# karenyang/GCN-VAE

Hardware: AMD Instinct MI355X
Metric: edges/sec R-GCN forward+backward, FB15k-237 emb=200 (higher is better)
Workload: dtype f32; 1 GPU; FB15k-237-shaped synthetic full graph (BASELINE configs[1]): 14541 entities, 474 directed relation types, E=544230 directed edges on this rank (544230 in the trained graph), 2-layer R-GCN-VAE bdd num_bases=100 emb_dim=200 dropout 0.2, 0 IAF blocks, DistMult decoder on T=220000 triplets per rank, step = fwd + loss(BCE+reg+KL+MMD) + bwd + clip + Adam; edges_per_gpu=544230, trained_graph_edges=544230, nodes=14541, triplets_per_gpu=220000, n_flows=0, gemm_precision=f32, launch=hipgraph, parallelism=single GPU, optimizer=replicated clip + Adam, k1_operands=f32

## Files before the change

### gcn-vae_amd/csrc/k_loss.hip

```cpp
#include "common.h"

namespace gv {

constexpr int RED_BLOCKS = 1024;

__device__ __forceinline__ float block_sum_256(float v, float* sm ) {
    v = wave_sum(v);
    const int lane = threadIdx.x & 63, w = threadIdx.x >> 6;
    __syncthreads();
    if (lane == 0) sm[w] = v;
    __syncthreads();
    return sm[0] + sm[1] + sm[2] + sm[3];
}

__global__ __launch_bounds__(256) void k_final_sum(const float* part, int n, float scale, float* out, int accumulate) {
    __shared__ float sm[4];
    float acc = 0.f;
    for (int i = threadIdx.x; i < n; i += 256) acc += part[i];
    const float tot = block_sum_256(acc, sm);
    if (threadIdx.x == 0) *out = accumulate ? *out + scale * tot : scale * tot;
}

__global__ __launch_bounds__(256) void k_loss_combine(const float* p0, int n0, float s0, const float* p1, int n1, float s1,
                                                      const float* p2, int n2, float s2, const float* p3, int n3, float s3,
// ... 1001 lines not shown
        } else {
            *reinterpret_cast<float4*>(o + 4 * q) = s4;
        }
    }
}

__global__ __launch_bounds__(256) void k_prior_sample_fwd(const float* z_pre, const float* eps, float* out, int s, int k, int h) {
    const int total = s * h;
    for (int i = blockIdx.x * 256 + threadIdx.x; i < total; i += gridDim.x * 256) {
        const int r = i / h, c = i - r * h, j = r % k;
        const float v = softplus_t(z_pre[(size_t)(k + j) * h + c]) + 1e-8f;
        out[i] = z_pre[(size_t)j * h + c] + eps[i] * sqrtf(v);
    }
}

__global__ __launch_bounds__(256) void k_prior_sample_bwd(const float* z_pre, const float* eps, const float* g, float* gz_pre,
                                                          int accumulate, int s, int k, int h) {
    const int total = k * h;
    for (int i = blockIdx.x * 256 + threadIdx.x; i < total; i += gridDim.x * 256) {
        const int j = i / h, c = i - j * h;
        const float raw = z_pre[(size_t)(k + j) * h + c];
        const float v = softplus_t(raw) + 1e-8f;
        float gm = 0.f, gs = 0.f;
        for (int r = j; r < s; r += k) {
            gm += g[(size_t)r * h + c];
            gs += g[(size_t)r * h + c] * eps[(size_t)r * h + c];
        }
        const float gr = gs * 0.5f / sqrtf(v) * (raw > 20.f ? 1.f : 1.f / (1.f + expf(-raw)));
        gz_pre[i] = accumulate ? gz_pre[i] + gm : gm;
        gz_pre[total + i] = accumulate ? gz_pre[total + i] + gr : gr;
    }
}

constexpr int KL_SLICES = 256;
constexpr int KL_FUSED_KT = 16;

}

using namespace gv;

#define GV_ST ((hipStream_t)stream)

static int red_blocks(int64_t n, int per_block) {
    int64_t b = (n + per_block - 1) / per_block;
    return (int)(b < 1 ? 1 : (b > RED_BLOCKS ? RED_BLOCKS : b));
}

static int sq2_blocks(int64_t n, int cap) {
    const int b = red_blocks(n, 4096);
    return b > cap ? cap : b;
}

static int kl_blocks(int64_t n) { return (int)((n + 3) / 4 > RED_BLOCKS ? RED_BLOCKS : (n + 3) / 4); }

extern "C" int gv_distmult_bce_fwd(const float* embed, int ld_e, const float* w_rel, int ld_w,
                                   const int32_t* triplets, const int32_t* order, const float* labels, const float* bias,
                                   float* score, float* loss, float* workspace, int64_t t, int h, void* stream) {
    GV_REQUIRE(embed && w_rel && triplets && labels && score && workspace, GV_ERR_NULL,
               "gv_distmult_bce_fwd: NULL pointer");
    GV_REQUIRE(t > 0 && h > 0 && ld_e >= h && ld_w >= h, GV_ERR_SHAPE, "gv_distmult_bce_fwd: bad shape");
    const int nb = red_blocks(t, 16);
    hipLaunchKernelGGL(k_distmult_bce, dim3(nb), dim3(256), 0, GV_ST, embed, ld_e, w_rel, ld_w, triplets, order, labels,
                       bias, score, workspace, t, h);
    if (loss) hipLaunchKernelGGL(k_final_sum, dim3(1), dim3(256), 0, GV_ST, workspace, nb, 1.f / (float)t, loss, 0);
    return launch_status("gv_distmult_bce_fwd");
}
// ... 250 lines not shown
    const float* kl_part = ws_kl ? ws_kl + 3 * (size_t)k * h : nullptr;
    hipLaunchKernelGGL(k_loss_combine, dim3(1), dim3(256), 0, GV_ST, ws_pred, n0, 1.f / (float)t, ws_reg, n1, 1.f, kl_part,
                       n2, ws_kl ? 1.f / (float)n_nodes : 0.f, ws_mmd, n3, 1.f, reg_w, kl_w, mmd_w, scal, loss, rows_dev,
                       (float)n_nodes);
    return launch_status("gv_loss_combine");
}

extern "C" int gv_mmd_bwd(const float* x, const float* y, const int64_t* y_index, int sx, int sy, int h, const float* gmmd,
                          float gscale, float* gx, float* gy, void* stream) {
    GV_REQUIRE(x && y && gx && gy, GV_ERR_NULL, "gv_mmd_bwd: NULL pointer");
    GV_REQUIRE(sx > 0 && sy > 0 && h > 0 && h <= 1024, GV_ERR_SHAPE, "gv_mmd_bwd: bad shape");
    static const int v2 = getenv("GV_MMD_ROWS16") ? atoi(getenv("GV_MMD_ROWS16")) : 1;
    const bool al = h % 4 == 0 && aligned16(x) && aligned16(y) && aligned16(gx) && aligned16(gy);
    if (v2 && al && h <= 256) hipLaunchKernelGGL(k_mmd_bwd_g<4>, dim3(sx + sy), dim3(64 * MMD_WAVES), 0, GV_ST, x, y, y_index, sx, sy, h, gmmd, gscale, gx, gy);
    else if (h <= 256) hipLaunchKernelGGL(k_mmd_bwd<4>, dim3(sx + sy), dim3(64 * MMD_WAVES), 0, GV_ST, x, y, y_index, sx, sy, h, gmmd, gscale, gx, gy);
    else hipLaunchKernelGGL(k_mmd_bwd<16>, dim3(sx + sy), dim3(64 * MMD_WAVES), 0, GV_ST, x, y, y_index, sx, sy, h, gmmd, gscale, gx, gy);
    return launch_status("gv_mmd_bwd");
}

extern "C" int gv_prior_sample_fwd(const float* z_pre, const float* eps, float* out, int s, int k, int h, void* stream) {
    GV_REQUIRE(z_pre && eps && out, GV_ERR_NULL, "gv_prior_sample_fwd: NULL pointer");
    GV_REQUIRE(s > 0 && k > 0 && h > 0, GV_ERR_SHAPE, "gv_prior_sample_fwd: bad shape");
    hipLaunchKernelGGL(k_prior_sample_fwd, dim3((s * h + 255) / 256), dim3(256), 0, GV_ST, z_pre, eps, out, s, k, h);
    return launch_status("gv_prior_sample_fwd");
}

extern "C" int gv_prior_sample_bwd(const float* z_pre, const float* eps, const float* g, float* gz_pre, int accumulate,
                                   int s, int k, int h, void* stream) {
    GV_REQUIRE(z_pre && eps && g && gz_pre, GV_ERR_NULL, "gv_prior_sample_bwd: NULL pointer");
    GV_REQUIRE(s > 0 && k > 0 && h > 0, GV_ERR_SHAPE, "gv_prior_sample_bwd: bad shape");
    hipLaunchKernelGGL(k_prior_sample_bwd, dim3((k * h + 255) / 256), dim3(256), 0, GV_ST, z_pre, eps, g, gz_pre, accumulate, s, k, h);
    return launch_status("gv_prior_sample_bwd");
}
```

### gcn-vae_amd/lib.py

```python
import ctypes
import os

import torch

_HERE = os.path.dirname(os.path.abspath(__file__))
LIB_PATH = os.path.join(_HERE, 'libgcnvae_hip.so')

_P, _I, _L, _F = ctypes.c_void_p, ctypes.c_int, ctypes.c_int64, ctypes.c_float

SIGNATURES = {
    'gv_version': (_I, []),
    'gv_last_error_string': (ctypes.c_char_p, []),
    'gv_index_caps': (None, [_L, _I, _I, _P, _P, _P]),
    'gv_index_workspace_bytes': (_L, [_L, _I]),
    'gv_build_csr': (_I, [_P, _L, _I, _I, _P, _P, _P, _I, _P, _I, _P, _L, _P]),
    'gv_build_csr_batch_workspace_bytes': (_L, [_P, _I]),
    'gv_build_csr_batch': (_I, [_P, _I, _P, _L, _P]),
    'gv_triplet_lists': (_I, [_P, _I, _L, _P, _P, _P, _P, _P, _P, _P, _P, _P]),
    'gv_widen2_i32': (_I, [_P, _P, _L, _P, _P, _L, _P]),
    'gv_graph_index_build': (_I, [_P, _P, _L, _I, _I, _I, _I, _P, _P, _P, _P, _I, _P, _I, _P, _P, _P, _P, _I, _P, _I, _P, _L, _P]),
    'gv_relation_index_build': (_I, [_P, _P, _P, _P, _P, _L, _I, _I, _P, _P, _P, _P, _P, _P, _P, _I, _P, _I, _P, _L, _P]),
    'gv_triplet_index_build': (_I, [_P, _L, _I, _I, _I, _I, _P, _P, _P, _P, _P, _I, _P, _I, _P, _P, _P, _P, _P, _I, _P, _I,
                                    _P, _L, _P]),
    'gv_perm_sample': (_I, [_L, _L, ctypes.c_uint64, ctypes.c_uint64, _P, _P, ctypes.c_uint32, _P, _P]),
# ... 76 lines not shown
    'gv_rank_scores': (_I, [_P, _I, _P, _I, _P, _P, _P, _P, _I, _I, _I, _P]),
    'gv_rank_scores_filtered': (_I, [_P, _I, _P, _I, _P, _P, _P, _P, _P, _I, _P, _P, _P, _I, _I, _I, _P]),
    'gv_topk_scores_workspace_bytes': (_L, [_I, _I, _I]),
    'gv_topk_scores': (_I, [_P, _I, _P, _I, _P, _P, _P, _P, _I, _I, _P, _P, _P, _I, _I, _I, _P]),
    'gv_rank_scores_constrained': (_I, [_P, _I, _P, _I, _P, _P, _P, _P, _P, _I, _P, _I, _I, _P, _P, _P, _P, _P, _P, _I, _I, _I, _P]),
    'gv_topk_scores_constrained': (_I, [_P, _I, _P, _I, _P, _P, _P, _P, _I, _P, _I, _I, _P, _I, _P, _P, _P, _I, _I, _I, _P]),
    'gv_mine_scores_workspace_bytes': (_L, [_I, _I, _I]),
    'gv_mine_scores': (_I, [_P, _I, _P, _I, _P, _P, _P, _P, _I, _I, _I, ctypes.c_uint32, _I, ctypes.c_uint32, _I, _P, _L, _P, _P, _P, _L,
                            _I, _I, _I, _P]),
    'gv_ec_basis_rows_fwd': (_I, [_P, _P, _P, _P, _L, _I, _I, _I, _L, _P, _P]),
    'gv_ec_basis_rows_bwd': (_I, [_P, _P, _P, _P, _P, _P, _L, _P, _P, _L, _I, _I, _I, _L, _P, _P, _P, _I, _P]),
    'gv_ec_head_fwd': (_I, [_P, _P, _P, _P, _L, _I, _P, _P, _P, _P, _P, _P]),
    'gv_ec_head_bwd': (_I, [_P, _P, _P, _P, _P, _P, _L, _I, _P, _P]),
    'gv_transe_sample': (_I, [_P, ctypes.c_uint32, _P, _L, _I, _P, _P, _P, _P, _P, _I, _I, _P, _P, _P, _P, _P]),
    'gv_transe_step': (_I, [_P, _P, _P, _P, _P, _I, _I, _I, _I, _I, _F, _F, _F, _P, _P, _P, _P, _P, _P]),
    'gv_transe_apply': (_I, [_P, _I, _P, _P, _P, _P, _I, _P, _P, _P, _I, _F, _P, _I, _F, _P, _P, _P]),
    'gv_transe_queries': (_I, [_P, _P, _P, _P, _L, _I, _I, _I, _P, _P]),
    'gv_transe_distances': (_I, [_P, _L, _P, _I, _I, _I, _P, _P]),
    'gv_transe_rank_filtered': (_I, [_P, _L, _P, _I, _I, _I, _P, _P, _P, _P, _P, _P, _P]),
    'gv_transe_topk_workspace_bytes': (_L, [_L, _I, _I]),
    'gv_transe_topk': (_I, [_P, _L, _P, _I, _I, _I, _P, _P, _P, _I, _I, _P, _P, _P, _P]),
    'gv_transe_rank_constrained': (_I, [_P, _L, _P, _I, _I, _I, _P, _P, _P, _P, _P, _I, _I, _P, _P, _P, _P, _P, _P]),
    'gv_transe_topk_constrained': (_I, [_P, _L, _P, _I, _I, _I, _P, _P, _P, _I, _P, _I, _I, _P, _I, _P, _P, _P, _P]),
    'gv_colsum': (_I, [_P, _P, _L, _I, _I, _P, _P, _I, _P]),
    'gv_gather_rows': (_I, [_P, _P, _P, _L, _I, _P]),
    'gv_gather_rows_rng_tick': (_I, [_P, _P, _P, _L, _I, _P, _P]),
    'gv_rng_fill': (_I, [_P, _I, _P, _P, _P, _P, _P, _P]),
    'gv_rng_tick': (_I, [_P, _P]),
    'gv_scatter_add_rows': (_I, [_P, _P, _P, _L, _I, _P]),
    'gv_reparam_fwd': (_I, [_P, _P, _P, _P, _P, _L, _I, _P]),
    'gv_reparam_bwd': (_I, [_P, _P, _P, _P, _P, _P, _P, _L, _I, _P]),
    'gv_distmult_bce_fwd': (_I, [_P, _I, _P, _I, _P, _P, _P, _P, _P, _P, _P, _L, _I, _P]),
    'gv_bce_grad': (_I, [_P, _P, _P, _P, _P, _P, _P, _P, _P, _L, _P]),
    'gv_mean_sq': (_I, [_P, _L, _F, _P, _P, _I, _P]),
    'gv_mean_sq2': (_I, [_P, _L, _F, _P, _L, _F, _P, _P, _P, _L, _P]),
    'gv_axpby': (_I, [_L, _P, _F, _P, _F, _P, _P]),
    'gv_mul': (_I, [_L, _P, _P, _P, _P]),
    'gv_mul_multi': (_I, [_I, _P, _P, _P, _P, _P]),
    'gv_kl_workspace_bytes': (_L, [_L, _I, _I]),
    'gv_kl_fwd': (_I, [_P, _P, _I, _P, _P, _P, _P, _P, _P, _L, _I, _I, _P, _P]),
    'gv_kl_bwd': (_I, [_P, _P, _I, _P, _P, _P, _P, _F, _F, _P, _P, _P, _P, _I, _P, _I, _L, _I, _I, _P, _P]),
    'gv_reparam_kl_fwd': (_I, [_P, _P, _P, _P, _P, _P, _P, _P, _L, _I, _I, _P]),
    'gv_reparam_kl_bwd': (_I, [_P, _P, _P, _P, _P, _P, _P, _F, _F, _P, _P, _P, _I, _P, _L, _I, _I, _P]),
    'gv_loss_combine': (_I, [_P, _L, _P, _L, _L, _P, _L, _I, _I, _P, _I, _I, _F, _F, _F, _P, _P, _P, _P]),
    'gv_lincomb4': (_I, [_P, _F, _P, _F, _P, _F, _P, _F, _P, _P]),
    'gv_mmd_fwd': (_I, [_P, _P, _P, _I, _I, _I, _P, _P, _P]),
    'gv_mmd_bwd': (_I, [_P, _P, _P, _I, _I, _I, _P, _F, _P, _P, _P]),
    'gv_prior_sample_fwd': (_I, [_P, _P, _P, _I, _I, _I, _P]),
    'gv_prior_sample_bwd': (_I, [_P, _P, _P, _P, _I, _I, _I, _I, _P]),
    'gv_iaf_update_fwd': (_I, [_P, _P, _I, _P, _P, _P, _L, _I, _P]),
    'gv_iaf_update_bwd': (_I, [_P, _P, _I, _P, _P, _P, _P, _P, _P, _L, _I, _P]),
    'gv_iaf_update_bwd_acc': (_I, [_P, _P, _I, _P, _P, _P, _P, _I, _P, _P, _L, _I, _P]),
    'gv_rowsum': (_I, [_P, _I, _I, _I, _P, _L, _P]),
    'gv_reverse_cols': (_I, [_P, _P, _L, _I, _P]),
    'gv_mean_rows_multi': (_I, [_I, _P, _L, _P, _P, _P, _P]),
    'gv_mean_rows_bwd': (_I, [_P, _L, _L, _P, _P, _P]),
    'gv_adam_step': (_I, [_P, _P, _P, _P, _L, _P, _F, _F, _F, _F, _F, _P, _P]),
    'gv_clip_adam_step': (_I, [_P, _P, _P, _P, _L, _P, _P, _F, _F, _F, _F, _F, _P, _I, _P]),
}

_lib = None
_fns = {}


def load():
    global _lib
# ... 59 lines not shown
```

### gcn-vae_amd/ops.py

```python
import contextlib
import ctypes as _ct
import itertools as _it
import os as _os
from dataclasses import dataclass
from typing import Optional

import torch

from . import lib
from .lib import ptr

ACT_NONE, ACT_RELU = 0, 1

DIRECT_GRAD = {}
GRAD_FRESH = set()
DIRECT_EPOCH = [0]


def _stamp_direct(ctx):
    ctx._gv_direct_epoch = DIRECT_EPOCH[0]


def _verify_direct(ctx):
    if getattr(ctx, '_gv_direct_epoch', DIRECT_EPOCH[0]) != DIRECT_EPOCH[0]:
# ... 1907 lines not shown
            d_zp = _direct_flat(z_pre)
            gzp = d_zp if d_zp is not None else torch.empty_like(z_pre)
            gh2 = torch.empty_like(h2)
            lib.call('gv_reparam_kl_bwd', ptr(z), ptr(h2), ptr(v), ptr(eps), ptr(z_pre), ptr(link.resp), ptr(link.gkl),
                     float(link.gscale), float(link.z_extra), ptr(gz), ptr(gh2), ptr(gzp), 1 if d_zp is not None else 0,
                     ptr(link.ws), n, h, z_pre.shape[0] // 2, lib.stream())
            link.gkl = None
            if gm is not None or gv is not None:
                extra = torch.empty_like(h2)
                gm = None if gm is None else _chk(gm.contiguous(), name='gm')
                gv = None if gv is None else _chk(gv.contiguous(), name='gv')
                lib.call('gv_reparam_bwd', ptr(h2), ptr(eps), ptr(v), None, ptr(gm), ptr(gv), ptr(extra), n, h, lib.stream())
                gh2 += extra
            return gh2, None, (None if d_zp is not None else gzp), None
        h2, eps, v = ctx.saved_tensors[:3]
        n, h = v.shape
        gz = None if gz is None else _chk(gz.contiguous(), name='gz')
        gm = None if gm is None else _chk(gm.contiguous(), name='gm')
        gv = None if gv is None else _chk(gv.contiguous(), name='gv')
        gh2 = torch.empty_like(h2)
        lib.call('gv_reparam_bwd', ptr(h2), ptr(eps), ptr(v), ptr(gz), ptr(gm), ptr(gv), ptr(gh2), n, h, lib.stream())
        return gh2, None, None, None


def reparam(h2, eps, z_pre=None):
    if z_pre is None or not FUSE_REPARAM_KL:
        return _Reparam.apply(h2, eps, None, None)
    box = [None]
    z, m, v = _Reparam.apply(h2, eps, z_pre, box)
    z._gv_kl_link = box[0]
    return z, m, v


class _DistMultBCE(torch.autograd.Function):

    @staticmethod
    def forward(ctx, embed, w_rel, bias, labels, tidx):
        ctx.set_materialize_grads(False)
        embed, ld_e = _row_major(embed, 'embed')
        w_rel, ld_w = _row_major(w_rel, 'w_relation')
        labels = _chk(labels.reshape(-1), name='labels')
        T, h = tidx.T, embed.shape[1]
        if labels.numel() != T:
            raise ValueError('labels / triplets length mismatch')
        score = torch.empty(T, dtype=torch.float32, device=embed.device)
        loss = torch.empty((), dtype=torch.float32, device=embed.device)
        ws = torch.empty(1024, dtype=torch.float32, device=embed.device)
        lib.call('gv_distmult_bce_fwd', ptr(embed), ld_e, ptr(w_rel), ld_w, ptr(tidx.trip32), ptr(tidx.fwd_order),
                 ptr(labels), ptr(bias), ptr(score), ptr(loss), ptr(ws), T, h, lib.stream())
        ctx.save_for_backward(embed, w_rel, labels, score)
        ctx.tidx, ctx.has_bias = tidx, bias is not None
        ctx.mark_non_differentiable(score)
        return loss, score

    @staticmethod
    def backward(ctx, gloss, _gscore):
        if gloss is None:
            return None, None, None, None, None
        embed, w_rel, labels, score = ctx.saved_tensors
        tidx = ctx.tidx
        T, h = tidx.T, embed.shape[1]
        dev = embed.device
        gloss = _chk(gloss.reshape(1).contiguous(), name='gloss')
        dscore = torch.empty(T, dtype=torch.float32, device=dev)
        dbias = torch.empty((), dtype=torch.float32, device=dev) if ctx.has_bias else None
        ws = torch.empty(1024, dtype=torch.float32, device=dev)
        lib.call('gv_bce_grad', ptr(score), ptr(labels), ptr(gloss), ptr(dscore), None, None, None, ptr(dbias), ptr(ws), T,
                 lib.stream())
        g_embed = g_w = None
        if ctx.needs_input_grad[0]:
            g_embed = bdd_aggregate(tidx.inc, tidx.inc_other, tidx.inc_rel, dscore, tidx.inc_tid, embed, w_rel,
                                    h, 1, 1)
        if ctx.needs_input_grad[1]:
            g_w = bdd_grad_weight(tidx.rel, tidx.rel_s, tidx.rel_o, dscore, tidx.rel_tid, embed, embed, h, 1, 1)
        return g_embed, g_w, dbias, None, None


def distmult_bce(embed, w_rel, bias, labels, tidx):
    return _DistMultBCE.apply(embed, w_rel, bias, labels, tidx)


class _DistMultScore(torch.autograd.Function):

    @staticmethod
    def forward(ctx, embed, w_rel, tidx):
        embed, ld_e = _row_major(embed, 'embed')
        w_rel, ld_w = _row_major(w_rel, 'w_relation')
        T, h = tidx.T, embed.shape[1]
        score = torch.empty(T, dtype=torch.float32, device=embed.device)
        loss = torch.empty((), dtype=torch.float32, device=embed.device)
        ws = torch.empty(1024, dtype=torch.float32, device=embed.device)
        zeros = torch.zeros(T, dtype=torch.float32, device=embed.device)
        lib.call('gv_distmult_bce_fwd', ptr(embed), ld_e, ptr(w_rel), ld_w, ptr(tidx.trip32), ptr(tidx.fwd_order), ptr(zeros),
                 None, ptr(score), ptr(loss), ptr(ws), T, h, lib.stream())
        ctx.save_for_backward(embed, w_rel)
        ctx.tidx = tidx
        return score

    @staticmethod
    def backward(ctx, gscore):
        embed, w_rel = ctx.saved_tensors
        tidx, h = ctx.tidx, embed.shape[1]
        gscore = _chk(gscore.contiguous(), name='gscore')
        g_embed = g_w = None
        if ctx.needs_input_grad[0]:
            g_embed = bdd_aggregate(tidx.inc, tidx.inc_other, tidx.inc_rel, gscore, tidx.inc_tid, embed, w_rel,
                                    h, 1, 1)
        if ctx.needs_input_grad[1]:
            g_w = bdd_grad_weight(tidx.rel, tidx.rel_s, tidx.rel_o, gscore, tidx.rel_tid, embed, embed, h, 1, 1)
        return g_embed, g_w, None


# ... 225 lines not shown
class _PriorSample(torch.autograd.Function):

    @staticmethod
    def forward(ctx, z_pre, eps):
        z_pre, eps = _chk(z_pre.contiguous(), name='z_pre'), _chk(eps.contiguous(), name='eps')
        k, h = z_pre.shape[0] // 2, z_pre.shape[1]
        out = torch.empty_like(eps)
        ctx.set_materialize_grads(False)
        lib.call('gv_prior_sample_fwd', ptr(z_pre), ptr(eps), ptr(out), eps.shape[0], k, h, lib.stream())
        ctx.save_for_backward(z_pre, eps)
        return out

    @staticmethod
    def backward(ctx, g):
        z_pre, eps = ctx.saved_tensors
        if g is None:
            return None, None
        g = _chk(g.contiguous(), name='g')
        d_zp = _direct_flat(z_pre)
        gz = d_zp if d_zp is not None else torch.empty_like(z_pre)
        lib.call('gv_prior_sample_bwd', ptr(z_pre), ptr(eps), ptr(g), ptr(gz), 1 if d_zp is not None else 0, eps.shape[0],
                 z_pre.shape[0] // 2, z_pre.shape[1], lib.stream())
        return (None if d_zp is not None else gz), None


def prior_sample(z_pre, eps):
    return _PriorSample.apply(z_pre, eps)


class _LossHead(torch.autograd.Function):

    @staticmethod
    def forward(ctx, z, z_mean, z_sigma, w_rel, z_pre, flp, z_pri, pick, labels, tidx, reg_w, kl_w, mmd_w, score_bias,
                embed_rows=None, rows_dev=None, kl_link=None):
        z, ld_z = _row_major(z, 'embed')
        if rows_dev is not None:
            rows_dev = _chk(rows_dev.reshape(-1), torch.int32, 'rows_dev')
            if kl_w <= 0 or embed_rows is not None:
                raise NotImplementedError('rows_dev needs kl_w > 0 (the padding rows are masked in the KL pass) and no embed_rows')
        w_rel, ld_w = _row_major(w_rel, 'w_relation')
        labels = _chk(labels.reshape(-1), name='labels')
        dev, (n, h), T = z.device, z.shape, tidx.T
        if labels.numel() != T:
            raise ValueError('labels / triplets length mismatch')
        f32 = dict(dtype=torch.float32, device=dev)
        ctx.set_materialize_grads(False)
        scal = torch.empty(4, **f32)
        pred, reg, kl, mmd = scal[0:1], scal[1:2], scal[2:3], scal[3:4]
        ws, ws2 = torch.empty(1024, **f32), torch.empty(1024, **f32)
        score = torch.empty(T, **f32)
        loss = torch.empty((), **f32)
        bias = flp if (score_bias and flp is not None) else None
        resp = wsk = z_post = wsm = None
        link = kl_link if (kl_link is not None and not kl_link.claimed and kl_w > 0 and flp is None and rows_dev is None
                           and embed_rows is None and kl_link.matches(z_pre) and kl_link.resp.shape[0] == n) else None
        if link is not None:
            link.claimed = True
        if kl_w > 0:
            z_mean, z_sigma = _chk(z_mean.contiguous(), name='z_mean'), _chk(z_sigma.contiguous(), name='z_sigma')
            z_pre = _chk(z_pre.contiguous(), name='z_pre')
            k = z_pre.shape[0] // 2
            if link is None:
                wsk = torch.empty(int(lib.load().gv_kl_workspace_bytes(n, h, k)) // 4, **f32)
                resp = torch.empty(n, k, **f32)
        if mmd_w > 0:
            z_pri = _chk(z_pri.contiguous(), name='z_pri')
            pick = _chk(pick.reshape(-1), torch.int64, 'pick')
            wsm = torch.empty(z_pri.shape[0] + pick.numel(), **f32)
        if ld_z != h or ld_w != h:
            raise ValueError('loss_head needs contiguous embeddings and relation table')
        st = lib.stream()
        if link is not None:
            resp, wsk = link.resp, link.ws
        elif kl_w > 0:
            lib.call('gv_kl_fwd', ptr(z), ptr(z_mean), h, ptr(z_sigma), ptr(z_pre), ptr(flp), ptr(resp), None, ptr(wsk),
                     n, h, k, ptr(rows_dev), st)
        if mmd_w > 0:
            lib.call('gv_mmd_fwd', ptr(z_pri), ptr(z), ptr(pick), z_pri.shape[0], pick.numel(), h, None, ptr(wsm), st)
        z_count = z.numel() if embed_rows is None else int(embed_rows) * h
        lib.call('gv_mean_sq2', ptr(z), z.numel(), 1.0 / z_count, ptr(w_rel), w_rel.numel(), 1.0 / w_rel.numel(), None,
                 ptr(ws2), ptr(rows_dev), n, st)
        lib.call('gv_distmult_bce_fwd', ptr(z), ld_z, ptr(w_rel), ld_w, ptr(tidx.trip32), ptr(tidx.fwd_order), ptr(labels),
                 ptr(bias), ptr(score), None, ptr(ws), T, h, st)
        lib.call('gv_loss_combine', ptr(ws), T, ptr(ws2), z.numel(), w_rel.numel(), ptr(wsk) if kl_w > 0 else None, n, h,
                 (z_pre.shape[0] // 2) if kl_w > 0 else 0, ptr(wsm) if mmd_w > 0 else None,
                 z_pri.shape[0] if mmd_w > 0 else 0, pick.numel() if mmd_w > 0 else 0, float(reg_w), float(kl_w),
                 float(mmd_w), ptr(scal), ptr(loss), ptr(rows_dev), st)
        ctx.save_for_backward(z, z_mean if kl_w > 0 else None, z_sigma if kl_w > 0 else None, w_rel,
                              z_pre if kl_w > 0 else None, resp, z_pri if mmd_w > 0 else None, z_post,
                              pick if mmd_w > 0 else None, labels, score, wsk, rows_dev)
        ctx.meta = (tidx, float(reg_w), float(kl_w), float(mmd_w), bias is not None, flp is not None and kl_w > 0)
        ctx.z_count = z_count
        ctx.kl_link = link
        ctx.direct_w = _direct(w_rel) if ld_w == h else None
        _stamp_direct(ctx)
        out_pred, out_kl, out_mmd = pred.reshape(()), kl.reshape(1), mmd.reshape(())
        ctx.mark_non_differentiable(out_pred, out_kl, out_mmd)
        return loss, out_pred, out_kl, out_mmd

    @staticmethod
    def backward(ctx, g, _gp, _gk, _gm):
        if g is None:
            return (None,) * 17
        z, z_mean, z_sigma, w_rel, z_pre, resp, z_pri, z_post, pick, labels, score, wsk, rows_dev = ctx.saved_tensors
        z_count = ctx.z_count
        tidx, reg_w, kl_w, mmd_w, has_bias, flp_in_kl = ctx.meta
        dev, (n, h), T = z.device, z.shape, tidx.T
        f32 = dict(dtype=torch.float32, device=dev)
        g = _chk(g.reshape(1).contiguous(), name='gloss')
        dscore = torch.empty(T, **f32)
        dbias = torch.empty((), **f32) if has_bias else None
        ws = torch.empty(1024, **f32)
        link = ctx.kl_link
        gz = torch.empty_like(z) if link is None else None
        gm = gv = gzp = d_zp = g_pri = g_post = None
        if link is not None:
            link.gkl, link.gscale, link.z_extra = g, kl_w, 2.0 * reg_w / z_count
            d_zp = True
        elif kl_w > 0:
            k = z_pre.shape[0] // 2
            d_zp = _direct_flat(z_pre)
            gm, gv = torch.empty_like(z), torch.empty_like(z)
            gzp = d_zp if d_zp is not None else torch.empty_like(z_pre)
        if mmd_w > 0:
            g_pri = torch.empty_like(z_pri)
        _verify_direct(ctx)
        d_w = ctx.direct_w
        g_w = d_w if d_w is not None else torch.empty_like(w_rel)
        g_flp = torch.empty((), **f32) if (has_bias or flp_in_kl) else None
        st = lib.stream()
        with fork(1):
            s1 = lib.stream()
            if link is not None:
                pass
            elif kl_w > 0:
                lib.call('gv_kl_bwd', ptr(z), ptr(z_mean), h, ptr(z_sigma), ptr(z_pre), ptr(resp), ptr(g), kl_w,
                         2.0 * reg_w / z_count, ptr(gz), ptr(gm), ptr(gv), ptr(gzp), 1 if d_zp is not None else 0, ptr(wsk),
                         1, n, h, k, ptr(rows_dev), s1)
            else:
                lib.call('gv_axpby', z.numel(), ptr(g), 2.0 * reg_w / z_count, ptr(z), 0.0, ptr(gz), s1)
            if mmd_w > 0 and link is None:
                lib.call('gv_mmd_bwd', ptr(z_pri), ptr(z), ptr(pick), z_pri.shape[0], pick.numel(), h, ptr(g), mmd_w,
                         ptr(g_pri), ptr(gz), s1)
        if tidx.pos3 is not None:
            d_inc, d_rel, idx_inc, idx_rel = torch.empty(2 * T, **f32), torch.empty(T, **f32), None, None
        else:
            d_inc, d_rel, idx_inc, idx_rel = dscore, dscore, tidx.inc_tid, tidx.rel_tid
        lib.call('gv_bce_grad', ptr(score), ptr(labels), ptr(g), ptr(dscore), ptr(tidx.pos3),
                 ptr(d_inc) if tidx.pos3 is not None else None, ptr(d_rel) if tidx.pos3 is not None else None,
                 ptr(dbias), ptr(ws), T, st)
        bdd_grad_weight(tidx.rel, tidx.rel_s, tidx.rel_o, d_rel, idx_rel, z, z, h, 1, 1, out=g_w,
                        accumulate=d_w is not None)
        lib.call('gv_axpby', w_rel.numel(), ptr(g), 2.0 * reg_w / w_rel.numel(), ptr(w_rel), 1.0, ptr(g_w), st)
        join(1)
        g_z = bdd_aggregate(indices.largest_first(tidx.inc) if indices.K1_ITEMS_LARGEST_FIRST else tidx.inc, tidx.inc_other, tidx.inc_rel,
                            d_inc, idx_inc, z, w_rel, h, 1, 1, addend=gz)
        if link is not None and mmd_w > 0:
            lib.call('gv_mmd_bwd', ptr(z_pri), ptr(z), ptr(pick), z_pri.shape[0], pick.numel(), h, ptr(g), mmd_w,
                     ptr(g_pri), ptr(g_z), st)
        if g_flp is not None:
            lib.call('gv_lincomb4', ptr(dbias) if has_bias else None, 1.0, ptr(g) if flp_in_kl else None, kl_w, None, 0.0,
                     None, 0.0, ptr(g_flp), st)
        return (g_z, gm, gv, (None if d_w is not None else g_w), (None if d_zp is not None else gzp), g_flp, g_pri, None,
                None, None, None, None, None, None, None, None, None)


def loss_head(z, z_mean, z_sigma, w_rel, z_pre, flp, z_pri, pick, labels, tidx, reg_w, kl_w, mmd_w, score_bias,
              embed_rows=None, rows_dev=None):
    return _LossHead.apply(z, z_mean, z_sigma, w_rel, z_pre, flp, z_pri, pick, labels, tidx, float(reg_w), float(kl_w),
                           float(mmd_w), bool(score_bias), embed_rows, rows_dev, getattr(z, '_gv_kl_link', None))


from .made import *
from .made import _ChainLayer, _RowLayer, _MADEForward, _MADEForwardBF16
from . import made


TRANSE_MAX_DIM = 512


def _i32(t, name, n=None):
    t = _chk(t, torch.int32, name)
    if not t.is_contiguous() or (n is not None and t.numel() != n):
        raise ValueError(f'{name}: expected a contiguous int32 tensor of {n} entries')
    return t


def _table(t, name):
    t = _chk(t, name=name)
    if t.dim() != 2 or not t.is_contiguous() or not 1 <= t.shape[1] <= TRANSE_MAX_DIM:
        raise ValueError(f'{name}: expected a contiguous (rows, dim) float32 table with 1 <= dim <= {TRANSE_MAX_DIM}')
    return t


def _p_norm(p):
    if p not in (1, 2):
        raise ValueError(f'p_norm must be 1 or 2, got {p}')
    return int(p)


def transe_sample(rng_state, stream_id, train, n_ent, batch, neg_ent, p_head=None, filt=None, bh=None, br=None, bt=None,
                  draws=None, check=True):
    train = _i32(train, 'train')
# ... 245 lines not shown
```

### include/gcnvae.h

```cpp
#ifndef GCNVAE_H
#define GCNVAE_H

#include <stdint.h>

#ifdef __cplusplus
extern "C" {
#endif

typedef enum {
    GV_OK = 0,
    GV_ERR_NULL = -1,
    GV_ERR_SHAPE = -2,
    GV_ERR_ALIGN = -3,
    GV_ERR_WORKSPACE = -4
} gv_status;

enum { GV_ACT_NONE = 0, GV_ACT_RELU = 1 };

int gv_version(void);
const char* gv_last_error_string(void);

int gv_segment_items_count(const int32_t* rowptr, int n_seg, int chunk, int32_t* n_chunks, int32_t* n_slots,
                           int32_t* is_split, void* stream);
int gv_segment_items_fill(const int32_t* rowptr, int n_seg, int chunk, const int32_t* item_off,
// ... 288 lines not shown
                       const uint64_t* c_tiles, int c_tiles_wanted, void* stream);
int gv_gemm_bf16(int trans_a, int trans_b, int m, int n, int k, const float* a, int lda, const float* b, int ldb,
                float* c, int ldc, const float* bias, int act, int accumulate, int split_k, const float* a_relu_mask,
                void* workspace, int64_t workspace_bytes, void* stream);

int gv_colsum(const float* x, const float* relu_mask, int64_t m, int n, int ld, float* out, float* workspace,
              int accumulate, void* stream);

int gv_gather_rows(const float* table, const int64_t* ids, float* out, int64_t n, int h, void* stream);
int gv_gather_rows_rng_tick(const float* table, const int64_t* ids, float* out, int64_t n, int h, uint64_t* rng_state,
                            void* stream);
int gv_scatter_add_rows(const float* grad_out, const int64_t* ids, float* grad_table, int64_t n, int h, void* stream);

#define GV_RNG_MAX_JOBS 8
#define GV_RNG_KEEP_MASK 0
#define GV_RNG_NORMAL 1
int gv_rng_fill(const uint64_t* rng_state, int n_jobs, void* const* ptrs, const int64_t* counts, const int32_t* kinds,
                const float* drop_p, const uint32_t* streams, void* stream);
int gv_rng_tick(uint64_t* rng_state, void* stream);

int gv_reparam_fwd(const float* h2, const float* eps, float* z, float* v, float* m_out ,
                   int64_t n, int h, void* stream);
int gv_reparam_bwd(const float* h2, const float* eps, const float* v, const float* gz, const float* gm,
                   const float* gv, float* grad_h2, int64_t n, int h, void* stream);

int gv_distmult_bce_fwd(const float* embed, int ld_e, const float* w_rel, int ld_w, const int32_t* triplets,
                        const int32_t* order ,
                        const float* labels, const float* bias, float* score, float* loss, float* workspace,
                        int64_t t, int h, void* stream);
int gv_bce_grad(const float* score, const float* labels, const float* gloss, float* dscore,
                const int32_t* pos3 , float* dscore_inc , float* dscore_rel ,
                float* dbias, float* workspace, int64_t t, void* stream);

int gv_mean_sq(const float* x, int64_t n, float scale, float* out, float* workspace, int accumulate, void* stream);
int gv_mean_sq2(const float* x1, int64_t n1, float scale1, const float* x2, int64_t n2, float scale2, float* out,
                float* workspace, const int32_t* rows_dev, int64_t rows_host, void* stream);
int gv_axpby(int64_t n, const float* a, float alpha, const float* x, float beta, float* y, void* stream);
int gv_mul(int64_t n, const float* a, const float* b, float* out, void* stream);
#define GV_MUL_MULTI_MAX 8
int gv_mul_multi(int count, const float* const* a, const float* const* b, float* const* out, const int64_t* n, void* stream);
int64_t gv_kl_workspace_bytes(int64_t n, int h, int k);
int gv_kl_fwd(const float* z, const float* m, int ld_m, const float* v, const float* z_pre, const float* flp,
              float* resp, float* kl, float* workspace, int64_t n, int h, int k, const int32_t* rows_dev, void* stream);
int gv_kl_bwd(const float* z, const float* m, int ld_m, const float* v, const float* z_pre, const float* resp,
              const float* gkl, float gscale, float z_extra, float* gz, float* gm, float* gv, float* g_zpre,
              int accumulate_zpre, float* workspace, int mix_ready, int64_t n, int h, int k, const int32_t* rows_dev,
              void* stream);
int gv_reparam_kl_fwd(const float* h2, const float* eps, const float* z_pre, float* z, float* v, float* m_out, float* resp,
                      float* workspace, int64_t n, int h, int k, void* stream);
int gv_reparam_kl_bwd(const float* z, const float* h2, const float* v, const float* eps, const float* z_pre, const float* resp,
                      const float* gkl, float gscale, float z_extra, const float* gz_up, float* gh2, float* g_zpre,
                      int accumulate_zpre, float* workspace, int64_t n, int h, int k, void* stream);

int gv_loss_combine(const float* ws_pred, int64_t t, const float* ws_reg, int64_t n_embed, int64_t n_wrel,
                    const float* ws_kl, int64_t n_nodes, int h, int k, const float* ws_mmd, int sx, int sy, float reg_w,
                    float kl_w, float mmd_w, float* scal , float* loss, const int32_t* rows_dev,
                    void* stream);
int gv_lincomb4(const float* a0, float c0, const float* a1, float c1, const float* a2, float c2, const float* a3,
                float c3, float* out, void* stream);
int gv_mmd_fwd(const float* x, const float* y, const int64_t* y_index, int sx, int sy, int h, float* mmd, float* workspace,
               void* stream);
int gv_mmd_bwd(const float* x, const float* y, const int64_t* y_index, int sx, int sy, int h, const float* gmmd, float gscale,
               float* gx, float* gy, void* stream);
int gv_prior_sample_fwd(const float* z_pre, const float* eps, float* out, int s, int k, int h, void* stream);
int gv_prior_sample_bwd(const float* z_pre, const float* eps, const float* g, float* gz_pre, int accumulate, int s, int k,
                        int h, void* stream);
// ... 86 lines not shown
```

Baseline: 551.8 million edges/s.

## Fuse DistMult BCE forward with relation-weight gradient sweep and finish kernel

Adds a fused kernel that computes DistMult scores, BCE loss, and the per-triplet sigmoid delta in one pass over the relation-sorted triplets. It also accumulates the relation-weight gradient partials (delta times s∘o) there, so the backward's separate bce_grad, bdd_grad_weight and axpby launches are replaced by one finish kernel that scales the partials, adds the L2 term, scales the coefficients and reduces dbias. This removes a second gather of subject/object embeddings over all triplets and several launches. In exchange the forward does extra gradient work and writes delta, u and partial buffers even if backward never runs. The path is gated by an env flag that defaults to on and falls back to the old kernels in no-grad mode.

```diff
diff --git a/gcn-vae_amd/csrc/k_loss.hip b/gcn-vae_amd/csrc/k_loss.hip
--- a/gcn-vae_amd/csrc/k_loss.hip
+++ b/gcn-vae_amd/csrc/k_loss.hip
@@ -1057,6 +1057,209 @@
     }
 }
 
+struct DmFusedParams {
+    const int4* items;
+    int n_items;
+    const int* rel_s;
+    const int* rel_o;
+    const int* rel_tid;
+    const float* e;
+    int ld_e;
+    const float* w;
+    int ld_w;
+    const float* labels;
+    const float* bias;
+    const int* pos3;
+    float* score;
+    float* delta;
+    float* u;
+    float* partial;
+    float* part;
+    int h;
+};
+
+constexpr int DM_PART = RED_BLOCKS;
+
+__device__ __forceinline__ int dm_rl_i(int v, int lane) { return __builtin_amdgcn_readlane(v, lane); }
+
+template <int U>
+__global__ __launch_bounds__(256) void k_distmult_bce_fwd_grad(const DmFusedParams a) {
+    __shared__ float sm[4];
+    const int lane = threadIdx.x & 63, wv = threadIdx.x >> 6;
+    const bool active = lane * 4 < a.h;
+    const int c0 = active ? lane * 4 : 0;
+    const float bv = a.bias ? *a.bias : 0.f;
+    const float* __restrict__ ebase = a.e + c0;
+    float lsum = 0.f, dsum = 0.f;
+    auto triplet = [&](const float (&xs)[4], const float (&xo)[4], const float (&wr)[4], float y, float (&acc)[4], float& x,
+                       float& d) {
+        float p[4];
+#pragma unroll
+        for (int i = 0; i < 4; ++i) p[i] = active ? xs[i] * xo[i] : 0.f;
+        float dot = p[0] * wr[0];
+        dot = fmaf(p[1], wr[1], dot);
+        dot = fmaf(p[2], wr[2], dot);
+        dot = fmaf(p[3], wr[3], dot);
+        x = wave_sum(dot) + bv;
+        d = 1.f / (1.f + expf(-x)) - y;
+#pragma unroll
+        for (int i = 0; i < 4; ++i) acc[i] = fmaf(d, p[i], acc[i]);
+    };
+    for (int quad = blockIdx.x; quad * 4 < a.n_items; quad += gridDim.x) {
+        const int item = __builtin_amdgcn_readfirstlane(quad * 4 + wv);
+        if (item >= a.n_items) continue;
+        const int4 it = a.items[item];
+        if (it.x < 0) continue;
+        if (it.w >= 0 && !a.partial) continue;
+        float wr[4] = {0.f, 0.f, 0.f, 0.f}, acc[4] = {0.f, 0.f, 0.f, 0.f};
+        if (active) load_vec<4>(a.w + (size_t)it.x * a.ld_w + c0, wr);
+        for (int e0 = it.y; e0 < it.z; e0 += 64) {
+            const int cnt = min(64, it.z - e0);
+            int my_s = 0, my_o = 0, my_t = 0;
+            float my_y = 0.f, my_x = 0.f, my_d = 0.f;
+            if (lane < cnt) {
+                my_s = a.rel_s[e0 + lane];
+                my_o = a.rel_o[e0 + lane];
+                my_t = a.rel_tid[e0 + lane];
+                my_y = a.labels[my_t];
+            }
+            int j = 0;
+            for (; j + U <= cnt; j += U) {
+                float xs[U][4], xo[U][4];
+#pragma unroll
+                for (int u = 0; u < U; ++u) {
+                    const int s = dm_rl_i(my_s, j + u), o = dm_rl_i(my_o, j + u);
+                    if (active) {
+                        load_vec<4>(ebase + (size_t)s * a.ld_e, xs[u]);
+                        load_vec<4>(ebase + (size_t)o * a.ld_e, xo[u]);
+                    }
+                }
+#pragma unroll
+                for (int u = 0; u < U; ++u) {
+                    float x, d;
+                    triplet(xs[u], xo[u], wr, rl_bcast_f(my_y, j + u), acc, x, d);
+                    if (lane == j + u) { my_x = x; my_d = d; }
+                }
+            }
+            for (; j < cnt; ++j) {
+                float xs[4], xo[4], x, d;
+                const int s = dm_rl_i(my_s, j), o = dm_rl_i(my_o, j);
+                if (active) {
+                    load_vec<4>(ebase + (size_t)s * a.ld_e, xs);
+                    load_vec<4>(ebase + (size_t)o * a.ld_e, xo);
+                }
+                triplet(xs, xo, wr, rl_bcast_f(my_y, j), acc, x, d);
+                if (lane == j) { my_x = x; my_d = d; }
+            }
+            if (lane < cnt) {
+                a.score[my_t] = my_x;
+                if (a.pos3) {
+                    a.delta[a.pos3[3 * (size_t)my_t]] = my_d;
+                    a.delta[a.pos3[3 * (size_t)my_t + 1]] = my_d;
+                } else {
+                    a.delta[my_t] = my_d;
+                }
+                lsum += fmaxf(my_x, 0.f) - my_x * my_y + log1pf(expf(-fabsf(my_x)));
+                dsum += my_d;
+            }
+        }
+        if (active) store_vec<4>((it.w >= 0 ? a.partial + (size_t)it.w * a.h : a.u + (size_t)it.x * a.h) + c0, acc);
+    }
+    const float lt = block_sum_256(lsum, sm);
+    const float dt = block_sum_256(dsum, sm);
+    if (threadIdx.x == 0) {
+        a.part[blockIdx.x] = lt;
+        a.part[DM_PART + blockIdx.x] = dt;
+    }
+}
+
+struct DmFinishParams {
+    const float* gloss;
+    const float* u;
+    const float* partial;
+    const int4* fix;
+    int n_fix;
+    const int* rowptr;
+    int chunk, num_rels, h;
+    const float* w;
+    int ld_w;
+    float reg_scale;
+    float* g_w;
+    int ld_gw, accumulate;
+    const float* delta;
+    float* d_out;
+    int64_t n_coef;
+    const float* part;
+    int n_part;
+    float* dbias;
+    int64_t t;
+    int nb_rows, nb_coef;
+};
+
+__global__ __launch_bounds__(256) void k_distmult_grad_finish(const DmFinishParams a) {
+    __shared__ float sm[4];
+    const float g = a.gloss ? *a.gloss : 1.f;
+    const float gt = g / (float)a.t;
+    const int b = blockIdx.x;
+    if (b < a.nb_rows) {
+        const int lane = threadIdx.x & 63;
+        const int n_rows = a.num_rels + a.n_fix;
+        const int row = b * 4 + (threadIdx.x >> 6);
+        if (row >= n_rows || lane * 4 >= a.h) return;
+        const int c0 = lane * 4;
+        int r;
+        float acc[4];
+        if (row < a.num_rels) {
+            r = row;
+            if (a.rowptr[r + 1] - a.rowptr[r] > a.chunk) return;
+            load_vec<4>(a.u + (size_t)r * a.h + c0, acc);
+        } else {
+            const int4 f = a.fix[row - a.num_rels];
+            if (f.x < 0) return;
+            r = f.x;
+            const float4* __restrict__ p = reinterpret_cast<const float4*>(a.partial + (size_t)f.y * a.h + c0);
+            const size_t stride = (size_t)(a.h >> 2);
+            float4 s[4];
+#pragma unroll
+            for (int i = 0; i < 4; ++i) s[i] = make_float4(0.f, 0.f, 0.f, 0.f);
+            int k = 0;
+            for (; k + 4 <= f.z; k += 4) {
+                float4 v[4];
+#pragma unroll
+                for (int i = 0; i < 4; ++i) v[i] = p[(size_t)(k + i) * stride];
+#pragma unroll
+                for (int i = 0; i < 4; ++i) { s[i].x += v[i].x; s[i].y += v[i].y; s[i].z += v[i].z; s[i].w += v[i].w; }
+            }
+            for (; k < f.z; ++k) {
+                const float4 v = p[(size_t)k * stride];
+                s[0].x += v.x; s[0].y += v.y; s[0].z += v.z; s[0].w += v.w;
+            }
+            acc[0] = (s[0].x + s[1].x) + (s[2].x + s[3].x);
+            acc[1] = (s[0].y + s[1].y) + (s[2].y + s[3].y);
+            acc[2] = (s[0].z + s[1].z) + (s[2].z + s[3].z);
+            acc[3] = (s[0].w + s[1].w) + (s[2].w + s[3].w);
+        }
+        float wr[4], out[4];
+        load_vec<4>(a.w + (size_t)r * a.ld_w + c0, wr);
+        float* o = a.g_w + (size_t)r * a.ld_gw + c0;
+        if (a.accumulate) load_vec<4>(o, out);
+#pragma unroll
+        for (int i = 0; i < 4; ++i) {
+            const float v = fmaf(gt, acc[i], g * a.reg_scale * wr[i]);
+            out[i] = a.accumulate ? out[i] + v : v;
+        }
+        store_vec<4>(o, out);
+    } else if (b < a.nb_rows + a.nb_coef) {
+        for (int64_t i = (int64_t)(b - a.nb_rows) * 256 + threadIdx.x; i < a.n_coef; i += (int64_t)a.nb_coef * 256)
+            a.d_out[i] = gt * a.delta[i];
+    } else {
+        float acc = 0.f;
+        for (int i = threadIdx.x; i < a.n_part; i += 256) acc += a.part[DM_PART + i];
+        const float tot = block_sum_256(acc, sm);
+        if (threadIdx.x == 0) *a.dbias = gt * tot;
+    }
+}
+
 constexpr int KL_SLICES = 256;
 constexpr int KL_FUSED_KT = 16;
 
@@ -1373,3 +1576,45 @@
     hipLaunchKernelGGL(k_prior_sample_bwd, dim3((k * h + 255) / 256), dim3(256), 0, GV_ST, z_pre, eps, g, gz_pre, accumulate, s, k, h);
     return launch_status("gv_prior_sample_bwd");
 }
+
+extern "C" int gv_distmult_bce_fwd_grad(const int32_t* items, int n_items, const int32_t* rel_s, const int32_t* rel_o,
+                                        const int32_t* rel_tid, const float* embed, int ld_e, const float* w_rel, int ld_w,
+                                        const float* labels, const float* bias, const int32_t* pos3, float* score,
+                                        float* delta, float* u, float* partial, float* workspace, int64_t t, int h,
+                                        void* stream) {
+    GV_REQUIRE(items && rel_s && rel_o && rel_tid && embed && w_rel && labels && score && delta && u && workspace,
+               GV_ERR_NULL, "gv_distmult_bce_fwd_grad: NULL pointer");
+    GV_REQUIRE(t > 0 && t < (1ll << 30) && n_items > 0, GV_ERR_SHAPE, "gv_distmult_bce_fwd_grad: t=%lld n_items=%d",
+               (long long)t, n_items);
+    GV_REQUIRE(h > 0 && h <= 256 && h % 4 == 0 && ld_e >= h && ld_w >= h && ld_e % 4 == 0 && ld_w % 4 == 0, GV_ERR_SHAPE,
+               "gv_distmult_bce_fwd_grad: h=%d (ld %d, %d): the fused sweep covers h <= 256, h %% 4 == 0", h, ld_e, ld_w);
+    GV_REQUIRE(aligned16(embed) && aligned16(w_rel) && aligned16(u) && aligned16(partial), GV_ERR_ALIGN,
+               "gv_distmult_bce_fwd_grad: 16-B alignment required");
+    DmFusedParams p{(const int4*)items, n_items, rel_s, rel_o, rel_tid, embed, ld_e, w_rel, ld_w, labels, bias, pos3,
+                    score, delta, u, partial, workspace, h};
+    hipLaunchKernelGGL(k_distmult_bce_fwd_grad<8>, dim3(red_blocks(t, 16)), dim3(256), 0, GV_ST, p);
+    return launch_status("gv_distmult_bce_fwd_grad");
+}
+
+extern "C" int gv_distmult_grad_finish(const float* gloss, const float* u, const float* partial, const int32_t* fix,
+                                       int n_fix, const int32_t* rowptr, int chunk, int num_rels, int h,
+                                       const float* w_rel, int ld_w, float reg_scale, float* grad_w, int ld_gw,
+                                       int accumulate, const float* delta, float* d_out, int64_t n_coef,
+                                       const float* workspace, float* dbias, int64_t t, void* stream) {
+    GV_REQUIRE(u && rowptr && w_rel && grad_w && delta && d_out, GV_ERR_NULL, "gv_distmult_grad_finish: NULL pointer");
+    GV_REQUIRE(n_fix == 0 || (fix && partial), GV_ERR_NULL, "gv_distmult_grad_finish: split rows need fix + partial");
+    GV_REQUIRE(!dbias || workspace, GV_ERR_NULL, "gv_distmult_grad_finish: dbias needs the forward's workspace");
+    GV_REQUIRE(t > 0 && n_coef > 0 && n_fix >= 0 && num_rels > 0 && chunk > 0, GV_ERR_SHAPE,
+               "gv_distmult_grad_finish: t=%lld n_coef=%lld n_fix=%d num_rels=%d chunk=%d", (long long)t, (long long)n_coef,
+               n_fix, num_rels, chunk);
+    GV_REQUIRE(h > 0 && h <= 256 && h % 4 == 0 && ld_w >= h && ld_gw >= h && ld_w % 4 == 0 && ld_gw % 4 == 0, GV_ERR_SHAPE,
+               "gv_distmult_grad_finish: h=%d (ld %d, %d): h <= 256, h %% 4 == 0", h, ld_w, ld_gw);
+    GV_REQUIRE(aligned16(u) && aligned16(partial) && aligned16(w_rel) && aligned16(grad_w), GV_ERR_ALIGN,
+               "gv_distmult_grad_finish: 16-B alignment required");
+    DmFinishParams p{gloss, u, partial, (const int4*)fix, n_fix, rowptr, chunk, num_rels, h, w_rel, ld_w, reg_scale, grad_w,
+                     ld_gw, accumulate, delta, d_out, n_coef, workspace, red_blocks(t, 16), dbias, t, 0, 0};
+    p.nb_rows = (num_rels + n_fix + 3) / 4;
+    p.nb_coef = red_blocks(n_coef, 1024);
+    hipLaunchKernelGGL(k_distmult_grad_finish, dim3(p.nb_rows + p.nb_coef + (dbias ? 1 : 0)), dim3(256), 0, GV_ST, p);
+    return launch_status("gv_distmult_grad_finish");
+}
diff --git a/gcn-vae_amd/lib.py b/gcn-vae_amd/lib.py
--- a/gcn-vae_amd/lib.py
+++ b/gcn-vae_amd/lib.py
@@ -132,6 +132,8 @@
     'gv_reparam_bwd': (_I, [_P, _P, _P, _P, _P, _P, _P, _L, _I, _P]),
     'gv_distmult_bce_fwd': (_I, [_P, _I, _P, _I, _P, _P, _P, _P, _P, _P, _P, _L, _I, _P]),
     'gv_bce_grad': (_I, [_P, _P, _P, _P, _P, _P, _P, _P, _P, _L, _P]),
+    'gv_distmult_bce_fwd_grad': (_I, [_P, _I, _P, _P, _P, _P, _I, _P, _I, _P, _P, _P, _P, _P, _P, _P, _P, _L, _I, _P]),
+    'gv_distmult_grad_finish': (_I, [_P, _P, _P, _P, _I, _P, _I, _I, _I, _P, _I, _F, _P, _I, _I, _P, _P, _L, _P, _P, _L, _P]),
     'gv_mean_sq': (_I, [_P, _L, _F, _P, _P, _I, _P]),
     'gv_mean_sq2': (_I, [_P, _L, _F, _P, _L, _F, _P, _P, _P, _L, _P]),
     'gv_axpby': (_I, [_L, _P, _F, _P, _F, _P, _P]),
diff --git a/gcn-vae_amd/ops.py b/gcn-vae_amd/ops.py
--- a/gcn-vae_amd/ops.py
+++ b/gcn-vae_amd/ops.py
@@ -1963,10 +1963,42 @@
     return z, m, v
 
 
+DISTMULT_FUSED = _os.environ.get('GV_DISTMULT_FUSED', '1') == '1'
+
+
+def distmult_fused_ok(embed, ld_e, w_rel, ld_w):
+    h = embed.shape[1]
+    return (DISTMULT_FUSED and h % 4 == 0 and h <= 256 and ld_e % 4 == 0 and ld_w % 4 == 0
+            and embed.data_ptr() % 16 == 0 and w_rel.data_ptr() % 16 == 0)
+
+
+def _distmult_fused_fwd(embed, ld_e, w_rel, ld_w, labels, bias, tidx, score, ws):
+    seg, T, h = tidx.rel, tidx.T, embed.shape[1]
+    _check_items(seg)
+    f32 = dict(dtype=torch.float32, device=embed.device)
+    delta = torch.empty(2 * T if tidx.pos3 is not None else T, **f32)
+    u = torch.empty(w_rel.shape[0], h, **f32)
+    partial = torch.empty(seg.n_slots, h, **f32) if seg.n_fix > 0 else None
+    lib.call('gv_distmult_bce_fwd_grad', ptr(seg.items), seg.n_items, ptr(tidx.rel_s), ptr(tidx.rel_o), ptr(tidx.rel_tid),
+             ptr(embed), ld_e, ptr(w_rel), ld_w, ptr(labels), ptr(bias), ptr(tidx.pos3), ptr(score), ptr(delta), ptr(u),
+             ptr(partial), ptr(ws), T, h, lib.stream())
+    return delta, u, partial
+
+
+def _distmult_fused_finish(fused, gloss, tidx, w_rel, ld_w, reg_scale, g_w, accumulate, ws, dbias):
+    delta, u, partial = fused
+    seg = tidx.rel
+    d_out = torch.empty_like(delta)
+    lib.call('gv_distmult_grad_finish', ptr(gloss), ptr(u), ptr(partial), ptr(seg.fix), seg.n_fix, ptr(seg.rowptr), seg.chunk,
+             w_rel.shape[0], w_rel.shape[1], ptr(w_rel), ld_w, float(reg_scale), ptr(g_w), g_w.stride(0), 1 if accumulate else 0,
+             ptr(delta), ptr(d_out), delta.numel(), ptr(ws), ptr(dbias), tidx.T, lib.stream())
+    return d_out
+
+
 class _DistMultBCE(torch.autograd.Function):
 
     @staticmethod
-    def forward(ctx, embed, w_rel, bias, labels, tidx):
+    def forward(ctx, embed, w_rel, bias, labels, tidx, grad_mode=True):
         ctx.set_materialize_grads(False)
         embed, ld_e = _row_major(embed, 'embed')
         w_rel, ld_w = _row_major(w_rel, 'w_relation')
@@ -1976,25 +2008,39 @@
             raise ValueError('labels / triplets length mismatch')
         score = torch.empty(T, dtype=torch.float32, device=embed.device)
         loss = torch.empty((), dtype=torch.float32, device=embed.device)
-        ws = torch.empty(1024, dtype=torch.float32, device=embed.device)
-        lib.call('gv_distmult_bce_fwd', ptr(embed), ld_e, ptr(w_rel), ld_w, ptr(tidx.trip32), ptr(tidx.fwd_order),
-                 ptr(labels), ptr(bias), ptr(score), ptr(loss), ptr(ws), T, h, lib.stream())
+        ws = torch.empty(2048, dtype=torch.float32, device=embed.device)
+        ctx.fused = None
+        if grad_mode and (ctx.needs_input_grad[0] or ctx.needs_input_grad[1]) and distmult_fused_ok(embed, ld_e, w_rel, ld_w):
+            ctx.fused = _distmult_fused_fwd(embed, ld_e, w_rel, ld_w, labels, bias, tidx, score, ws)
+            lib.call('gv_loss_combine', ptr(ws), T, None, 0, 0, None, 0, h, 0, None, 0, 0, 0.0, 0.0, 0.0, None, ptr(loss), None,
+                     lib.stream())
+        else:
+            lib.call('gv_distmult_bce_fwd', ptr(embed), ld_e, ptr(w_rel), ld_w, ptr(tidx.trip32), ptr(tidx.fwd_order),
+                     ptr(labels), ptr(bias), ptr(score), ptr(loss), ptr(ws), T, h, lib.stream())
         ctx.save_for_backward(embed, w_rel, labels, score)
-        ctx.tidx, ctx.has_bias = tidx, bias is not None
+        ctx.tidx, ctx.has_bias, ctx.ws, ctx.ld_w = tidx, bias is not None, ws, ld_w
         ctx.mark_non_differentiable(score)
         return loss, score
 
     @staticmethod
     def backward(ctx, gloss, _gscore):
         if gloss is None:
-            return None, None, None, None, None
+            return None, None, None, None, None, None
         embed, w_rel, labels, score = ctx.saved_tensors
         tidx = ctx.tidx
         T, h = tidx.T, embed.shape[1]
         dev = embed.device
         gloss = _chk(gloss.reshape(1).contiguous(), name='gloss')
+        dbias = torch.empty((), dtype=torch.float32, device=dev) if ctx.has_bias else None
+        if ctx.fused is not None:
+            g_w = torch.empty_like(w_rel)
+            d_inc = _distmult_fused_finish(ctx.fused, gloss, tidx, w_rel, ctx.ld_w, 0.0, g_w, False, ctx.ws, dbias)
+            g_embed = None
+            if ctx.needs_input_grad[0]:
+                g_embed = bdd_aggregate(tidx.inc, tidx.inc_other, tidx.inc_rel, d_inc,
+                                        None if tidx.pos3 is not None else tidx.inc_tid, embed, w_rel, h, 1, 1)
+            return g_embed, (g_w if ctx.needs_input_grad[1] else None), dbias, None, None, None
         dscore = torch.empty(T, dtype=torch.float32, device=dev)
-        dbias = torch.empty((), dtype=torch.float32, device=dev) if ctx.has_bias else None
         ws = torch.empty(1024, dtype=torch.float32, device=dev)
         lib.call('gv_bce_grad', ptr(score), ptr(labels), ptr(gloss), ptr(dscore), None, None, None, ptr(dbias), ptr(ws), T,
                  lib.stream())
@@ -2004,11 +2050,11 @@
                                     h, 1, 1)
         if ctx.needs_input_grad[1]:
             g_w = bdd_grad_weight(tidx.rel, tidx.rel_s, tidx.rel_o, dscore, tidx.rel_tid, embed, embed, h, 1, 1)
-        return g_embed, g_w, dbias, None, None
+        return g_embed, g_w, dbias, None, None, None
 
 
 def distmult_bce(embed, w_rel, bias, labels, tidx):
-    return _DistMultBCE.apply(embed, w_rel, bias, labels, tidx)
+    return _DistMultBCE.apply(embed, w_rel, bias, labels, tidx, torch.is_grad_enabled())
 
 
 class _DistMultScore(torch.autograd.Function):
@@ -2300,7 +2346,7 @@
 
     @staticmethod
     def forward(ctx, z, z_mean, z_sigma, w_rel, z_pre, flp, z_pri, pick, labels, tidx, reg_w, kl_w, mmd_w, score_bias,
-                embed_rows=None, rows_dev=None, kl_link=None):
+                embed_rows=None, rows_dev=None, kl_link=None, grad_mode=True):
         z, ld_z = _row_major(z, 'embed')
         if rows_dev is not None:
             rows_dev = _chk(rows_dev.reshape(-1), torch.int32, 'rows_dev')
@@ -2315,7 +2361,7 @@
         ctx.set_materialize_grads(False)
         scal = torch.empty(4, **f32)
         pred, reg, kl, mmd = scal[0:1], scal[1:2], scal[2:3], scal[3:4]
-        ws, ws2 = torch.empty(1024, **f32), torch.empty(1024, **f32)
+        ws, ws2 = torch.empty(2048, **f32), torch.empty(1024, **f32)
         score = torch.empty(T, **f32)
         loss = torch.empty((), **f32)
         bias = flp if (score_bias and flp is not None) else None
@@ -2348,8 +2394,13 @@
         z_count = z.numel() if embed_rows is None else int(embed_rows) * h
         lib.call('gv_mean_sq2', ptr(z), z.numel(), 1.0 / z_count, ptr(w_rel), w_rel.numel(), 1.0 / w_rel.numel(), None,
                  ptr(ws2), ptr(rows_dev), n, st)
-        lib.call('gv_distmult_bce_fwd', ptr(z), ld_z, ptr(w_rel), ld_w, ptr(tidx.trip32), ptr(tidx.fwd_order), ptr(labels),
-                 ptr(bias), ptr(score), None, ptr(ws), T, h, st)
+        ctx.fused = None
+        if grad_mode and (ctx.needs_input_grad[0] or ctx.needs_input_grad[3]) and distmult_fused_ok(z, ld_z, w_rel, ld_w):
+            ctx.fused = _distmult_fused_fwd(z, ld_z, w_rel, ld_w, labels, bias, tidx, score, ws)
+            ctx.ws = ws
+        else:
+            lib.call('gv_distmult_bce_fwd', ptr(z), ld_z, ptr(w_rel), ld_w, ptr(tidx.trip32), ptr(tidx.fwd_order), ptr(labels),
+                     ptr(bias), ptr(score), None, ptr(ws), T, h, st)
         lib.call('gv_loss_combine', ptr(ws), T, ptr(ws2), z.numel(), w_rel.numel(), ptr(wsk) if kl_w > 0 else None, n, h,
                  (z_pre.shape[0] // 2) if kl_w > 0 else 0, ptr(wsm) if mmd_w > 0 else None,
                  z_pri.shape[0] if mmd_w > 0 else 0, pick.numel() if mmd_w > 0 else 0, float(reg_w), float(kl_w),
@@ -2369,16 +2420,17 @@
     @staticmethod
     def backward(ctx, g, _gp, _gk, _gm):
         if g is None:
-            return (None,) * 17
+            return (None,) * 18
         z, z_mean, z_sigma, w_rel, z_pre, resp, z_pri, z_post, pick, labels, score, wsk, rows_dev = ctx.saved_tensors
         z_count = ctx.z_count
         tidx, reg_w, kl_w, mmd_w, has_bias, flp_in_kl = ctx.meta
         dev, (n, h), T = z.device, z.shape, tidx.T
         f32 = dict(dtype=torch.float32, device=dev)
         g = _chk(g.reshape(1).contiguous(), name='gloss')
-        dscore = torch.empty(T, **f32)
+        fused = ctx.fused
+        dscore = torch.empty(T, **f32) if fused is None else None
         dbias = torch.empty((), **f32) if has_bias else None
-        ws = torch.empty(1024, **f32)
+        ws = torch.empty(1024, **f32) if fused is None else None
         link = ctx.kl_link
         gz = torch.empty_like(z) if link is None else None
         gm = gv = gzp = d_zp = g_pri = g_post = None
@@ -2410,16 +2462,21 @@
             if mmd_w > 0 and link is None:
                 lib.call('gv_mmd_bwd', ptr(z_pri), ptr(z), ptr(pick), z_pri.shape[0], pick.numel(), h, ptr(g), mmd_w,
                          ptr(g_pri), ptr(gz), s1)
-        if tidx.pos3 is not None:
-            d_inc, d_rel, idx_inc, idx_rel = torch.empty(2 * T, **f32), torch.empty(T, **f32), None, None
+        if fused is not None:
+            d_inc = _distmult_fused_finish(fused, g, tidx, w_rel, h, 2.0 * reg_w / w_rel.numel(), g_w, d_w is not None, ctx.ws,
+                                           dbias)
+            idx_inc = None if tidx.pos3 is not None else tidx.inc_tid
         else:
-            d_inc, d_rel, idx_inc, idx_rel = dscore, dscore, tidx.inc_tid, tidx.rel_tid
-        lib.call('gv_bce_grad', ptr(score), ptr(labels), ptr(g), ptr(dscore), ptr(tidx.pos3),
-                 ptr(d_inc) if tidx.pos3 is not None else None, ptr(d_rel) if tidx.pos3 is not None else None,
-                 ptr(dbias), ptr(ws), T, st)
-        bdd_grad_weight(tidx.rel, tidx.rel_s, tidx.rel_o, d_rel, idx_rel, z, z, h, 1, 1, out=g_w,
-                        accumulate=d_w is not None)
-        lib.call('gv_axpby', w_rel.numel(), ptr(g), 2.0 * reg_w / w_rel.numel(), ptr(w_rel), 1.0, ptr(g_w), st)
+            if tidx.pos3 is not None:
+                d_inc, d_rel, idx_inc, idx_rel = torch.empty(2 * T, **f32), torch.empty(T, **f32), None, None
+            else:
+                d_inc, d_rel, idx_inc, idx_rel = dscore, dscore, tidx.inc_tid, tidx.rel_tid
+            lib.call('gv_bce_grad', ptr(score), ptr(labels), ptr(g), ptr(dscore), ptr(tidx.pos3),
+                     ptr(d_inc) if tidx.pos3 is not None else None, ptr(d_rel) if tidx.pos3 is not None else None,
+                     ptr(dbias), ptr(ws), T, st)
+            bdd_grad_weight(tidx.rel, tidx.rel_s, tidx.rel_o, d_rel, idx_rel, z, z, h, 1, 1, out=g_w,
+                            accumulate=d_w is not None)
+            lib.call('gv_axpby', w_rel.numel(), ptr(g), 2.0 * reg_w / w_rel.numel(), ptr(w_rel), 1.0, ptr(g_w), st)
         join(1)
         g_z = bdd_aggregate(indices.largest_first(tidx.inc) if indices.K1_ITEMS_LARGEST_FIRST else tidx.inc, tidx.inc_other, tidx.inc_rel,
                             d_inc, idx_inc, z, w_rel, h, 1, 1, addend=gz)
@@ -2430,13 +2487,14 @@
             lib.call('gv_lincomb4', ptr(dbias) if has_bias else None, 1.0, ptr(g) if flp_in_kl else None, kl_w, None, 0.0,
                      None, 0.0, ptr(g_flp), st)
         return (g_z, gm, gv, (None if d_w is not None else g_w), (None if d_zp is not None else gzp), g_flp, g_pri, None,
-                None, None, None, None, None, None, None, None, None)
+                None, None, None, None, None, None, None, None, None, None)
 
 
 def loss_head(z, z_mean, z_sigma, w_rel, z_pre, flp, z_pri, pick, labels, tidx, reg_w, kl_w, mmd_w, score_bias,
               embed_rows=None, rows_dev=None):
     return _LossHead.apply(z, z_mean, z_sigma, w_rel, z_pre, flp, z_pri, pick, labels, tidx, float(reg_w), float(kl_w),
-                           float(mmd_w), bool(score_bias), embed_rows, rows_dev, getattr(z, '_gv_kl_link', None))
+                           float(mmd_w), bool(score_bias), embed_rows, rows_dev, getattr(z, '_gv_kl_link', None),
+                           torch.is_grad_enabled())
 
 
 from .made import *
diff --git a/include/gcnvae.h b/include/gcnvae.h
--- a/include/gcnvae.h
+++ b/include/gcnvae.h
@@ -344,6 +344,15 @@
                 const int32_t* pos3 , float* dscore_inc , float* dscore_rel ,
                 float* dbias, float* workspace, int64_t t, void* stream);
 
+int gv_distmult_bce_fwd_grad(const int32_t* items, int n_items, const int32_t* rel_s, const int32_t* rel_o,
+                             const int32_t* rel_tid, const float* embed, int ld_e, const float* w_rel, int ld_w,
+                             const float* labels, const float* bias, const int32_t* pos3, float* score, float* delta,
+                             float* u, float* partial, float* workspace, int64_t t, int h, void* stream);
+int gv_distmult_grad_finish(const float* gloss, const float* u, const float* partial, const int32_t* fix, int n_fix,
+                            const int32_t* rowptr, int chunk, int num_rels, int h, const float* w_rel, int ld_w,
+                            float reg_scale, float* grad_w, int ld_gw, int accumulate, const float* delta, float* d_out,
+                            int64_t n_coef, const float* workspace, float* dbias, int64_t t, void* stream);
+
 int gv_mean_sq(const float* x, int64_t n, float scale, float* out, float* workspace, int accumulate, void* stream);
 int gv_mean_sq2(const float* x1, int64_t n1, float scale1, const float* x2, int64_t n2, float scale2, float* out,
                 float* workspace, const int32_t* rows_dev, int64_t rows_host, void* stream);
```

Measured after the change: 569.8 million edges/s (median of 6 runs). +3.3%, better.
